# B-R-P/NMSLIB-ZIG

Hardware: AMD Instinct MI355X
Metric: queries/sec @ recall@10, 1M x 128-D L2, batch=1024; HBM GB/s vs peak (higher is better)
Workload: dtype f16+f32

## Files before the change

nmslib_zig_amd/csrc/kernels/bf_kernels.hip:

```cpp
#include <cstdio>
#include <type_traits>
#include <vector>
#include <cstdlib>

#include "common_dev.hpp"
#include "kernels.hpp"

namespace gfxknn {

enum BfMode : int { BF_L2 = 0, BF_DOT = 1, BF_COS = 2, BF_L1 = 3, BF_LINF = 4, BF_COSC = 5, BF_L2D = 6 };

struct BfArgs {
    const float* base;
    const float* aux;
    const float* qaux;
    int aux_stride;
    const float* queries;
    u64* cand;
    int* cand_cnt;
    uint32_t* gthr;
    uint32_t* gq;
    int xj, xm;
    int n, ldb, nqt, nsplit, rows_per_split, kprime, cap;
    int kcs;
// ... 752 lines not shown
            check_block(acc1, 1, t - 1);
        }
        __builtin_amdgcn_sched_barrier(0);
        if (!compute) break;
        const bool more = t + kRing - 1 < nstages;
        if (more && !(a.dbg & 2)) issue_tile(t + kRing - 1);
#pragma unroll
        for (int i = 0; i < 16; ++i) {
            acc0[i] = 0;
            acc1[i] = 0;
        }
#pragma unroll
        for (int ks = 0; ks < 4; ++ks) {
            acc0 = __builtin_amdgcn_mfma_i32_32x32x32_i8(fa[ks], bq[ks], acc0, 0, 0, 0);
            acc1 = __builtin_amdgcn_mfma_i32_32x32x32_i8(fb[ks], bq[ks], acc1, 0, 0, 0);
        }
        if (a.dbg & 1) asm volatile("" ::"v"(acc0[0]), "v"(acc1[0]), "v"(acc0[15]), "v"(acc1[15]));
        if (a.xj > 0 && !(a.dbg & 256) && t > 0 && (((t - 1) & t) == 0 || ((t - 1) & 31) == 31)) exchange_counted();
        if (a.dbg & 8) continue;
        if (more) asm volatile("s_waitcnt vmcnt(12)\n\ts_barrier" ::: "memory");
        else asm volatile("s_waitcnt vmcnt(0)\n\ts_barrier" ::: "memory");
    }
    if (nstages > 0 && !(a.dbg & 1)) {
        if (a.xj > 0 && !(a.dbg & 256)) exchange_counted();
        finish_stage(true);
    }
    if (h == 0) a.cand_cnt[(size_t)qidx * a.nsplit + split] = mycnt;
}

__device__ __forceinline__ uint32_t hit_mask_f32(const f32x16& c, float t) {
    typedef float f32x2 __attribute__((ext_vector_type(2)));
    uint32_t m = 0u;
    const f32x2 tt = {t, t};
#pragma unroll
    for (int i0 = 0; i0 < 16; i0 += 8) {
        f32x2 d[4];
#pragma unroll
        for (int j = 0; j < 4; ++j) d[j] = f32x2{c[i0 + 2 * j], c[i0 + 2 * j + 1]} - tt;
        asm volatile("" : "+v"(d[0]), "+v"(d[1]), "+v"(d[2]), "+v"(d[3]));
#pragma unroll
        for (int j = 0; j < 4; ++j) {
            m = __builtin_amdgcn_alignbit(m, __float_as_uint(d[j][0]), 31);
            m = __builtin_amdgcn_alignbit(m, __float_as_uint(d[j][1]), 31);
        }
    }
    return ~m & 0xffffu;
}
__device__ __forceinline__ uint32_t hit_mask_i32(const i32x16& c, int t) {
    uint32_t m = 0u;
#pragma unroll
    for (int i = 0; i < 16; ++i) m = __builtin_amdgcn_alignbit(m, (uint32_t)(c[i] - t), 31);
    return ~m & 0xffffu;
}
__device__ __forceinline__ void scan_gather_entries(u64* keys, const int* offs, const uint32_t* list, int q, int nl, int caph,
                                                    int tps, int tid, int nthreads) {
    for (int s = tid; s < nl; s += nthreads) {
        const int len = offs[s + 1] - offs[s];
        if (len == 0) continue;
        const uint32_t* e = list + (size_t)q * caph * nl + s;
        const uint32_t row_base = (uint32_t)(s >> 1) * (uint32_t)tps * BF_BN + 4u * (s & 1);
        uint32_t pre[4];
#pragma unroll
        for (int i = 0; i < 4; ++i) pre[i] = (i < len && i < caph) ? e[(size_t)i * nl] : 0u;
        int j = 0;
        auto expand = [&](const uint32_t ent) __attribute__((always_inline)) {
            uint32_t m = ent & 0xffffu;
            const uint32_t r0 = row_base + (ent >> 16) * 32u;
            while (m && j < len) {
                const int bit = 31 - __builtin_clz(m);
                m &= ~(1u << bit);
                const int reg = 15 - bit;
                keys[offs[s] + j++] = (u64)(r0 + (reg & 3) + 8 * (reg >> 2));
            }
        };
#pragma unroll
        for (int i = 0; i < 4; ++i)
            if (i < caph && j < len) expand(pre[i]);
        for (int i = 4; i < caph && j < len; ++i) expand(e[(size_t)i * nl]);
    }
}

struct BfScanArgs {
    const uint8_t* base_i8;
    const int32_t* auxh;
    const uint8_t* queries;
    const int* thr;
    uint32_t* list;
    int* list_cnt;
    int n, nqt, nsplit, tps, caph;
    int tile_stride;
    int* top8;
};

template <int QG, bool SAMPLE>
__global__ __launch_bounds__(256, 2) void bf_scan_u8_kernel(BfScanArgs a) {
    extern __shared__ __attribute__((aligned(16))) char smem[];
    const int tid = threadIdx.x, lane = tid & 63, wave = tid >> 6;
    const int h = lane >> 5, l31 = lane & 31;
    const int b = blockIdx.x;
    const int xcd = b & 7, rest = b >> 3;
    const int qt = rest % a.nqt;
    const int split = (rest / a.nqt) * 8 + xcd;
    if (split >= a.nsplit) return;

    constexpr int kGroup = 4, kRing = 2 * kGroup, kAuxRing = 8, kTileBytes = BF_BN * 128;
    char* ring = smem;
    int* auxr = reinterpret_cast<int*>(ring + kRing * kTileBytes);

    const int tstr = SAMPLE ? a.tile_stride : 1;
    const int tiles_all = (a.n + BF_BN - 1) / BF_BN;
    const int stiles_all = (tiles_all + tstr - 1) / tstr;
    const int nstages = max(0, min(a.tps, stiles_all - split * a.tps));
    const int r_begin = split * a.tps * tstr * BF_BN;
    const int stage_rows = tstr * BF_BN;

    const int dma_row = lane >> 3;
    uint32_t dma_voff[2];
#pragma unroll
    for (int jj = 0; jj < 2; ++jj) {
        const int row = 8 * (2 * wave + jj) + dma_row;
        dma_voff[jj] = (uint32_t)(row * 128 + ((lane & 7) ^ ((row >> 1) & 7)) * 16);
    }
    const uint32_t dma_lds0 = (uint32_t)(uintptr_t)(lptr_t)ring + (uint32_t)(2 * __builtin_amdgcn_readfirstlane(wave) * 1024);
    const uint32_t aux_lds0 = (uint32_t)(uintptr_t)(lptr_t)auxr;
    const uint32_t aux_voff = (uint32_t)lane * 4u;
    auto issue_tile = [&](int stage) __attribute__((always_inline)) {
        const int slot = stage % kRing;
        const int row0 = r_begin + stage * stage_rows;
        const unsigned long long sbase = (unsigned long long)(uintptr_t)a.base_i8 + (unsigned long long)row0 * 128ull;
        const uint32_t m0v = dma_lds0 + (uint32_t)slot * kTileBytes;
#pragma clang diagnostic push
// ... 259 lines not shown
                bsq = __builtin_amdgcn_udot4(bv[u][t], bv[u][t], bsq, false);
                dot = __builtin_amdgcn_udot4(bv[u][t], qv[t], dot, false);
            }
            int d = qsq + bsq - 2 * dot;
            d += __shfl_xor(d, 1, 64);
            d += __shfl_xor(d, 2, 64);
            d += __shfl_xor(d, 4, 64);
            const int j = j0 + 8 * u + g8;
            if (sub == 0 && j < total) keys[j] = ((u64)i32_ord(d) << 32) | pos[u];
        }
    }
    for (int i = total + tid; i < P; i += blockDim.x) keys[i] = ~0ull;
    __syncthreads();
    block_bitonic_u64_asc(keys, P, tid, blockDim.x);
    const int found = total < a.k ? total : a.k;
    for (int i = tid; i < a.k; i += blockDim.x) {
        int32_t id = -1;
        float d = INFINITY;
        if (i < found) {
            const u64 key = keys[i];
            const uint32_t pos = (uint32_t)key;
            id = a.ext_ids ? a.ext_ids[pos] : (int32_t)pos;
            d = (float)ord_i32((uint32_t)(key >> 32));
        }
        a.out_ids[(size_t)q * a.k + i] = id;
        a.out_dists[(size_t)q * a.k + i] = d;
    }
    if (tid == 0 && a.out_cnt) a.out_cnt[q] = found;
}

typedef __bf16 bf16x8 __attribute__((ext_vector_type(8)));
typedef _Float16 f16x8 __attribute__((ext_vector_type(8)));

enum ScanMode : int { SC_L2 = 0, SC_DOT = 1, SC_COS = 2 };

struct BfScanF32Args {
    const __bf16* base_hi;
    const __bf16* base_lo;
    const float* auxp;
    const __bf16* q_hi;
    const __bf16* q_lo;
    const void* base_h16;
    const void* q_h16;
    const float* auxp16;
    int prio_half;
    const float* thr;
    uint32_t* list;
    int* list_cnt;
    int n, nqt, nsplit, tps, caph;
    int tile_stride;
    float* top8;
    const int* group_flag;
    int group_want;
};

#define BF_FRAG_RD(REGS, var, addr) asm volatile("ds_read_b128 %0, %1" : "={" REGS "}"(var) : "v"(addr) : "memory")
#define BF_FRAG_RD_OFF(REGS, var, addr, off) \
    asm volatile("ds_read_b128 %0, %1 offset:%2" : "={" REGS "}"(var) : "v"(addr), "n"(off) : "memory")

template <int MODE, bool SAMPLE, int QG>
__global__ __launch_bounds__(256) void bf_scan_f32_kernel(BfScanF32Args a) {
    constexpr int NW = 4;
    extern __shared__ __attribute__((aligned(16))) char smem[];
    const int tid = threadIdx.x, lane = tid & 63, wave = tid >> 6;
    const int h = lane >> 5, l31 = lane & 31;
    const int b = blockIdx.x;
    const int xcd = b & 7, rest = b >> 3;
    const int qt = rest % a.nqt;
    const int split = (rest / a.nqt) * 8 + xcd;
    if (split >= a.nsplit) return;
    if (a.group_flag && (a.group_flag[qt] != 0) != (a.group_want != 0)) return;

    constexpr int kRing = 4, kAuxRing = 8, kHalfBytes = BF_BN * 256, kStageBytes = 2 * kHalfBytes;
    char* ring = smem;
    float* auxr = reinterpret_cast<float*>(ring + kRing * kStageBytes);

    const int tstr = SAMPLE ? a.tile_stride : 1;
    const int tiles_all = (a.n + BF_BN - 1) / BF_BN;
    const int stiles_all = (tiles_all + tstr - 1) / tstr;
    const int nstages = max(0, min(a.tps, stiles_all - split * a.tps));
    const int r_begin = split * a.tps * tstr * BF_BN;
    const int stage_rows = tstr * BF_BN;

    constexpr int kPieces = 32 / NW;
    static_assert(kPieces == 8, "a wave's pieces lie in one half of the stage");
    const int wave_u = __builtin_amdgcn_readfirstlane(wave);
    uint32_t dma_voff[kPieces];
#pragma unroll
    for (int jj = 0; jj < kPieces; ++jj) {
        const int pj = (kPieces * wave + jj) & 15;
        const int row = 4 * pj + (lane >> 4);
        dma_voff[jj] = (uint32_t)((row * 128 + ((lane & 15) ^ (row & 15)) * 8) * 2);
    }
    const int dma_half = (kPieces * wave_u) >> 4;
    const uint32_t dma_lds0 = (uint32_t)(uintptr_t)(lptr_t)ring + (uint32_t)(dma_half * kHalfBytes + ((kPieces * wave_u) & 15) * 1024);
    const unsigned long long dma_src0 = (unsigned long long)(uintptr_t)(dma_half ? a.base_lo : a.base_hi);
    const uint32_t aux_lds0 = (uint32_t)(uintptr_t)(lptr_t)auxr;
    const uint32_t aux_voff = (uint32_t)lane * 4u;
    auto issue_tile = [&](int stage) __attribute__((always_inline)) {
        const int slot = stage % kRing;
        const int row0 = r_begin + stage * stage_rows;
        const unsigned long long sbase = dma_src0 + (unsigned long long)row0 * 256ull;
        const uint32_t m0v = dma_lds0 + (uint32_t)slot * kStageBytes;
#pragma clang diagnostic push
#pragma clang diagnostic ignored "-Winline-asm"
#pragma unroll
// ... 312 lines not shown
        if constexpr (MODE == SC_COS) return c[i] * ax[(i & 3) + 8 * (i >> 2)];
        else return c[i];
    };
    auto block_max_leaves = [&](const f32x16& c, const float* ax, float (&m)[5]) __attribute__((always_inline)) {
#pragma unroll
        for (int j = 0; j < 5; ++j) {
            if constexpr (MODE == SC_COS)
                m[j] = fmaxf(fmaxf(score_of(c, 3 * j, ax), score_of(c, 3 * j + 1, ax)), score_of(c, 3 * j + 2, ax));
            else
                asm("v_max3_f32 %0, %1, %2, %3" : "=v"(m[j]) : "v"(c[3 * j]), "v"(c[3 * j + 1]), "v"(c[3 * j + 2]));
        }
    };
    auto block_max_root = [&](const f32x16& c, const float* ax, const float (&m)[5]) __attribute__((always_inline)) -> float {
        if constexpr (MODE == SC_COS) {
            return fmaxf(fmaxf(fmaxf(m[0], m[1]), m[2]), fmaxf(fmaxf(m[3], m[4]), score_of(c, 15, ax)));
        } else {
            float r0, r1, r;
            asm("v_max3_f32 %0, %1, %2, %3" : "=v"(r0) : "v"(m[0]), "v"(m[1]), "v"(m[2]));
            asm("v_max3_f32 %0, %1, %2, %3" : "=v"(r1) : "v"(m[3]), "v"(m[4]), "v"(c[15]));
            asm("v_max_f32 %0, %1, %2" : "=v"(r) : "v"(r0), "v"(r1));
            return r;
        }
    };
    auto block_max = [&](const f32x16& c, const float* ax) __attribute__((always_inline)) -> float {
        float m[5];
        block_max_leaves(c, ax, m);
        return block_max_root(c, ax, m);
    };
    auto trigger_of = [&](float m, int g) __attribute__((always_inline)) -> unsigned long long {
        return SAMPLE ? __builtin_amdgcn_ballot_w64(m > thr[g]) : __builtin_amdgcn_ballot_w64(m >= thr[g]);
    };
    auto finish_check = [&](unsigned long long trig, float m, const f32x16& c, int g, const float* ax, int row0) __attribute__((always_inline)) {
        if constexpr (SAMPLE) {
            if (__builtin_expect(trig != 0ull, 0)) {
                float v = (row0 + 32 <= a.n || MODE == SC_L2) ? m : -INFINITY;
#pragma unroll
                for (int j = 0; j < 8; ++j) {
                    const float hi = fmaxf(t8[g][j], v);
                    v = fminf(t8[g][j], v);
                    t8[g][j] = hi;
                }
                thr[g] = t8[g][7];
            }
        } else if (__builtin_expect(trig != 0ull, 0)) {
            uint32_t km;
            if constexpr (MODE == SC_COS) {
                f32x16 sc;
#pragma unroll
                for (int i = 0; i < 16; ++i) sc[i] = score_of(c, i, ax);
                km = hit_mask_f32(sc, thr[g]);
            } else {
                km = hit_mask_f32(c, thr[g]);
            }
            if (row0 + 32 > a.n) {
                int nvalid = a.n - row0;
                asm volatile("" : "+s"(nvalid));
#pragma unroll
                for (int i = 0; i < 16; ++i)
                    if (acc_row(i, h) >= nvalid) km &= ~(0x8000u >> i);
            }
            if (km) {
                if (ecnt[g] < a.caph) lp[g][(size_t)ecnt[g] * (2 * a.nsplit)] = ((uint32_t)(row0 - r_begin) >> 5 << 16) | km;
                ecnt[g]++;
                cnt[g] += __builtin_popcount(km);
            }
        }
    };

    f16x8 fh[4];
    f32x16 iv;
#pragma unroll
    for (int i = 0; i < 16; ++i) iv[i] = 0.f;
    f32x16 acc[2][QG];
#pragma unroll
    for (int g = 0; g < QG; ++g) {
#pragma unroll
        for (int i = 0; i < 16; ++i) {
            acc[0][g][i] = 0.f;
            acc[1][g][i] = -INFINITY;
        }
    }
    const float* pv_ax = auxr;
    int pv_row0 = 0;
    bool have_pv = false;
    float m_pend = 0.f;
    unsigned long long trig_pend = 0ull;
    const uint32_t lds0 = (uint32_t)(uintptr_t)(lptr_t)smem;
    auto load_frag = [&](auto off_tag, int kc) __attribute__((always_inline)) {
        constexpr int OFF = decltype(off_tag)::value;
        const uint32_t ad = vad[kc];
        if constexpr (NW == 4) {
            switch (kc % 4) {
                case 0: BF_FRAG_RD_OFF("v[224:227]", fh[0], ad, OFF); break;
                case 1: BF_FRAG_RD_OFF("v[228:231]", fh[1], ad, OFF); break;
                case 2: BF_FRAG_RD_OFF("v[232:235]", fh[2], ad, OFF); break;
                default: BF_FRAG_RD_OFF("v[236:239]", fh[3], ad, OFF); break;
            }
        } else {
            switch (kc % 4) {
                case 0: BF_FRAG_RD_OFF("v[96:99]", fh[0], ad, OFF); break;
                case 1: BF_FRAG_RD_OFF("v[100:103]", fh[1], ad, OFF); break;
                case 2: BF_FRAG_RD_OFF("v[104:107]", fh[2], ad, OFF); break;
                default: BF_FRAG_RD_OFF("v[108:111]", fh[3], ad, OFF); break;
            }
        }
    };
    using Off0 = std::integral_constant<int, 0>;
    using Off1 = std::integral_constant<int, 32 * 256>;
    auto wait_frag = [&](auto cnt_tag, int kc, bool with_init) __attribute__((always_inline)) {
        constexpr int N = decltype(cnt_tag)::value;
#define BF_W1(STR)                                                                                              \
        if constexpr (NW == 4) {                                                                                \
            switch (kc % 4) {                                                                                   \
                case 0:                                                                                         \
                    if (with_init) asm volatile(STR : "+{v[224:227]}"(fh[0]), "+{v[240:255]}"(iv));             \
// ... 263 lines not shown
#pragma unroll
        for (int i = 0; i < NPER; ++i) {
            const float v = ord_f32(key[i]);
            const bool c = key[i] != 0u && key[i] <= T && v > -INFINITY && t3 - v >= need;
            best = c && key[i] > best ? key[i] : best;
        }
#pragma unroll
        for (int o = 32; o > 0; o >>= 1) {
            const uint32_t other = (uint32_t)__shfl_xor((int)best, o, 64);
            best = other > best ? other : best;
        }
        ok = false;
        if (best != 0u) {
            int above = 0;
#pragma unroll
            for (int i = 0; i < NPER; ++i) above += __popcll(__builtin_amdgcn_ballot_w64(key[i] > best));
            const int jmax = rcap < total ? rcap : total;
            const int j = best == T ? r : above + 1;
            if (j <= jmax) {
                t1 = ord_f32(best);
                ok = true;
            }
        }
    }
    if (lane == 0) {
        thr3[q] = (t3 - 1.02f * e1) / unit;
        thr1[q] = force_precise == 2 ? INFINITY : t1;
        if (!ok) atomicOr(&precise[q / group_q], 1);
    }
}

struct RerankListF32Args {
    const float* base;
    const float* queries;
    const uint32_t* list;
    const int* list_cnt;
    const int32_t* ext_ids;
    int32_t* out_ids;
    float* out_dists;
    int32_t* out_cnt;
    int* tile_fail;
    int n, k, nsplit, caph, p2max, fail_queries, space, dim, ldb;
    int tps;
    const float* queries_sel;
    const float* thr;
    const float* thr1;
    const int* precise;
    int no_split;
    float bmax;
    float bres;
    float scale, scale_q, bres16;
    int sel_dim, sel_ld;
    const float* qaux;
    unsigned long long* prof;
};

__global__ __launch_bounds__(256) void bf_rerank_f32_list_kernel(RerankListF32Args a) {
    const unsigned long long t0 = a.prof ? wall_clock64() : 0;
    auto lap = [&](int i) __attribute__((always_inline)) {
        if (a.prof && threadIdx.x == 0) atomicAdd(&a.prof[i], wall_clock64() - t0);
    };
    extern __shared__ __attribute__((aligned(16))) char smem[];
    u64* keys = reinterpret_cast<u64*>(smem);
    int* offs = reinterpret_cast<int*>(keys + a.p2max);
    __shared__ int s_over, s_split;
    __shared__ float s_qn2, s_e1, s_thr;
    const int q = blockIdx.x, tid = threadIdx.x, lane = tid & 63, wave = tid >> 6;
    const int nl = 2 * a.nsplit;
    if (tid == 0) s_over = 0;
    __syncthreads();
    if (tid < 64) {
        const int per = (nl + 63) / 64;
        int sum = 0, over = 0;
        for (int i = 0; i < per; ++i) {
            const int s = tid * per + i;
            if (s < nl) {
                const int c = a.list_cnt[(size_t)q * nl + s];
                over |= c > a.caph;
                sum += c < a.caph ? c : a.caph;
            }
        }
        int incl = sum;
#pragma unroll
        for (int o = 1; o < 64; o <<= 1) {
            const int v = __shfl_up(incl, o, 64);
            if (tid >= o) incl += v;
        }
        int run = incl - sum;
        for (int i = 0; i < per; ++i) {
            const int s = tid * per + i;
            if (s < nl) {
                offs[s] = run;
                const int c = a.list_cnt[(size_t)q * nl + s];
                run += c < a.caph ? c : a.caph;
            }
        }
        if (tid == 63) offs[nl] = incl;
        if (__any(over != 0) && tid == 0) s_over = 1;
    } else if (wave == 1) {
        const bool split_product = a.precise[q / a.fail_queries] != 0;
        const float* qs = a.queries_sel + (size_t)q * a.sel_ld;
        float ss = 0.f;
        for (int d = lane; d < a.sel_dim; d += 64) ss = fmaf(qs[d], qs[d], ss);
        ss = wave_sum(ss);
        const float e1 = split_product ? 0.f : one_product_error(qs, a.sel_dim, lane, a.scale * (a.space == SP_L2 || a.space == SP_NEGDOT || a.qaux ? a.bmax : 1.0f), a.bres16, a.scale_q);
        if (lane == 0) {
            s_qn2 = ss;
            s_e1 = e1;
            s_split = split_product ? 1 : 0;
            s_thr = split_product ? a.thr[q] : a.thr1[q];
        }
    }
    __syncthreads();
    const int total = offs[nl];
    if ((a.no_split && a.precise[q / a.fail_queries] != 0) ||
        (a.qaux && a.qaux[(size_t)q * 4 + 3] == 0.f)) {
        if (tid == 0) atomicOr(&a.tile_fail[q / a.fail_queries], 1);
        return;
    }
    const int need = a.k < a.n ? a.k : a.n;
    const int want = need + (a.k / 8 > 4 ? a.k / 8 : 4) < a.n ? need + (a.k / 8 > 4 ? a.k / 8 : 4) : a.n;
    if (s_over || total < want || total > a.p2max) {
        if (tid == 0) atomicOr(&a.tile_fail[q / a.fail_queries], 1);
        return;
    }
    lap(0);
    scan_gather_entries(keys, offs, a.list, q, nl, a.caph, a.tps, tid, blockDim.x);
    __syncthreads();
    lap(1);
    const int P = next_pow2(total < 2 ? 2 : total);
    if (a.prof && tid == 0) {
        atomicAdd(&a.prof[8], (unsigned long long)total);
        atomicAdd(&a.prof[9], (unsigned long long)P);
        atomicAdd(&a.prof[10], 1ull);
    }
    const float* qq = a.queries + (size_t)q * a.ldb;
    const int sub = lane & 15, rg = lane >> 4;
    if (a.dim <= 128) {
        float qv[8];
        bool ok[8];
    #pragma unroll
        for (int c = 0; c < 8; ++c) {
            const int d = sub + 16 * c;
            ok[c] = d < a.dim;
            qv[c] = ok[c] ? qq[d] : 0.f;
        }
        constexpr int kU = 4;
        for (int j0 = wave * (4 * kU); j0 < total; j0 += 16 * kU) {
            uint32_t pos[kU];
            float xv[kU][8];
    #pragma unroll
            for (int u = 0; u < kU; ++u) {
                const int j = j0 + 4 * u + rg;
                pos[u] = (uint32_t)keys[j < total ? j : total - 1];
                const float* row = a.base + (size_t)pos[u] * a.ldb + sub;
    #pragma unroll
                for (int c = 0; c < 8; ++c) xv[u][c] = ok[c] ? row[16 * c] : 0.f;
            }
            __builtin_amdgcn_wave_barrier();
    #pragma unroll
            for (int u = 0; u < kU; ++u) {
                float p0[4], p1[4], p2[4];
    #pragma unroll
                for (int v = 0; v < 4; ++v) {
                    p0[v] = p1[v] = p2[v] = 0.f;
    #pragma unroll
                    for (int c = 0; c < 2; ++c) {
                        if (64 * c >= a.dim) continue;
                        const float x = xv[u][v + 4 * c], y = qv[v + 4 * c];
                        if (a.space == SP_L2) {
                            const float t = x - y;
                            p0[v] = fmaf(t, t, p0[v]);
                        } else {
                            p0[v] = fmaf(x, y, p0[v]);
                            if (a.space != SP_NEGDOT) {
                                p1[v] = fmaf(x, x, p1[v]);
                                p2[v] = fmaf(y, y, p2[v]);
                            }
                        }
                    }
                }
                auto tree = [&](const float* p) __attribute__((always_inline)) -> float {
                    float s = (p[0] + p[2]) + (p[1] + p[3]);
    #pragma unroll
                    for (int o = 8; o > 0; o >>= 1) s += __shfl_xor(s, o, 64);
                    return s;
                };
// ... 82 lines not shown
    }
    __syncthreads();
    lap(2);
    if (total <= 512 && a.k <= 32) {
        __shared__ u64 s_head[128];
        const int e0 = wave * 128 + 2 * lane;
        u64 k0 = e0 < total ? keys[e0] : ~0ull, k1 = e0 + 1 < total ? keys[e0 + 1] : ~0ull;
        wave_sort128_u64(k0, k1, lane);
        if (lane < 16) {
            s_head[wave * 32 + 2 * lane] = k0;
            s_head[wave * 32 + 2 * lane + 1] = k1;
        }
        __syncthreads();
        if (wave == 0) {
            k0 = s_head[2 * lane];
            k1 = s_head[2 * lane + 1];
            wave_sort128_u64(k0, k1, lane);
            if (lane < 16) {
                keys[2 * lane] = k0;
                keys[2 * lane + 1] = k1;
            }
        }
        __syncthreads();
    } else {
        for (int i = total + tid; i < P; i += blockDim.x) keys[i] = ~0ull;
        __syncthreads();
        block_bitonic_u64_asc(keys, P, tid, blockDim.x);
    }
    lap(3);
    const int found = total < a.k ? total : a.k;
    if (total < a.n) {
        const bool split_product = s_split != 0;
        if (tid == 0) {
            const float qn2 = s_qn2, qn = sqrtf(qn2);
            const float dk = ord_f32((uint32_t)(keys[found - 1] >> 32));
            float sk, e, extra = 0.f;
            if (a.qaux) {
                const float sh = sinf(0.5f * dk);
                const float omc = a.space == SP_ANGULAR ? 2.0f * sh * sh : dk;
                const float qnorm = a.qaux[(size_t)q * 4 + 2];
                sk = -omc * qnorm;
                e = 6.1036e-5f * qn * a.bmax;
                extra = 1e-6f * qn * a.bmax + 2e-6f * qnorm;
            } else if (a.space == SP_L2) {
                sk = 0.5f * (qn2 - dk * dk);
                e = 6.1036e-5f * qn * a.bmax;
            } else if (a.space == SP_NEGDOT) {
                sk = -dk;
                e = 6.1036e-5f * qn * a.bmax;
            } else {
                sk = (a.space == SP_ANGULAR ? cosf(dk) : 1.0f - dk) * qn;
                e = 6.1036e-5f * qn;
            }
            const float t = s_thr;
            if (!split_product) {
                const float unit = a.scale * a.scale_q;
                sk *= unit;
                extra *= unit;
                e = s_e1;
            }
            e += extra + 1e-6f * (fabsf(sk) + fabsf(t));
            if (!(sk - t >= e)) atomicOr(&a.tile_fail[q / a.fail_queries], 1);
        }
    }
    lap(4);
    for (int i = tid; i < a.k; i += blockDim.x) {
        int32_t id = -1;
        float d = INFINITY;
        if (i < found) {
            const u64 key = keys[i];
            const uint32_t pos = (uint32_t)key;
            id = a.ext_ids ? a.ext_ids[pos] : (int32_t)pos;
            d = ord_f32((uint32_t)(key >> 32));
        }
        a.out_ids[(size_t)q * a.k + i] = id;
        a.out_dists[(size_t)q * a.k + i] = d;
    }
    if (tid == 0 && a.out_cnt) a.out_cnt[q] = found;
    lap(5);
}

__global__ void row_maxnorm_kernel(const float* rows, int n, int ld, int dim, int relative, unsigned* out_bits, float scale16) {
    const int lane = threadIdx.x & 63;
    const int wpb = blockDim.x >> 6;
    float mb = 0.f, mr = 0.f, ma = 0.f, mh = 0.f;
    for (int row = blockIdx.x * wpb + (threadIdx.x >> 6); row < n; row += gridDim.x * wpb) {
        const float* p = rows + (size_t)row * ld;
        float s = 0.f, r = 0.f, rh = 0.f;
        for (int d = lane; d < dim; d += 64) {
            const float v = p[d], w = v - (float)(__bf16)v;
            const float vs = scale16 * v, wh = vs - (float)(_Float16)vs;
            s = fmaf(v, v, s);
            r = fmaf(w, w, r);
            rh = fmaf(wh, wh, rh);
            ma = fmaxf(ma, fabsf(v));
        }
        s = wave_sum(s);
        r = wave_sum(r);
        rh = wave_sum(rh);
        const float nb = sqrtf(s), nr = sqrtf(r), nh = sqrtf(rh);
        mb = fmaxf(mb, nb);
        mr = fmaxf(mr, relative ? (nb > 0.f ? nr / nb : 0.f) : nr);
        mh = fmaxf(mh, relative ? (nb > 0.f ? nh / nb : 0.f) : nh);
    }
    ma = wave_max(ma);
    if (lane == 0) {
        atomicMax(out_bits, __float_as_uint(mb));
// ... 929 lines not shown
}

template <int MODE, bool SAMPLE, int QG>
static hipError_t launch_scan_f32_one(const BfScanF32Args& a, int grid, size_t lds, hipStream_t s) {
    hipError_t e = hipFuncSetAttribute(reinterpret_cast<const void*>(bf_scan_f32_kernel<MODE, SAMPLE, QG>),
                                       hipFuncAttributeMaxDynamicSharedMemorySize, (int)lds);
    if (e != hipSuccess) return e;
    hipLaunchKernelGGL((bf_scan_f32_kernel<MODE, SAMPLE, QG>), dim3(grid), dim3(256), lds, s, a);
    return hipGetLastError();
}
template <int MODE, bool SAMPLE, int QG, int NW>
static hipError_t launch_scan_bf16_one(const BfScanF32Args& a, int grid, size_t lds, hipStream_t s) {
    hipError_t e = hipFuncSetAttribute(reinterpret_cast<const void*>(bf_scan_bf16_kernel<MODE, SAMPLE, QG, NW>),
                                       hipFuncAttributeMaxDynamicSharedMemorySize, (int)lds);
    if (e != hipSuccess) return e;
    hipLaunchKernelGGL((bf_scan_bf16_kernel<MODE, SAMPLE, QG, NW>), dim3(grid), dim3(NW * 64), lds, s, a);
    return hipGetLastError();
}
template <int MODE>
static hipError_t launch_scan_f32_mode(const BfScanF32Args& a, bool sample, int terms, int qg, int grid, size_t lds, hipStream_t s, int kch = 1) {
    if (kch > 1) {
        if (terms != 1) return hipSuccess;
        auto go = [&](auto kern) -> hipError_t {
            hipError_t e = hipFuncSetAttribute(reinterpret_cast<const void*>(kern), hipFuncAttributeMaxDynamicSharedMemorySize, (int)lds);
            if (e != hipSuccess) return e;
            hipLaunchKernelGGL(kern, dim3(grid), dim3(256), lds, s, a);
            return hipGetLastError();
        };
        switch (kch) {
            case 2: return sample ? go(bf_scan_bf16_kernel<MODE, true, 1, 4, 2>) : go(bf_scan_bf16_kernel<MODE, false, 1, 4, 2>);
            case 3: return sample ? go(bf_scan_bf16_kernel<MODE, true, 1, 4, 3>) : go(bf_scan_bf16_kernel<MODE, false, 1, 4, 3>);
            case 4: return sample ? go(bf_scan_bf16_kernel<MODE, true, 1, 4, 4>) : go(bf_scan_bf16_kernel<MODE, false, 1, 4, 4>);
            case 6: return sample ? go(bf_scan_bf16_kernel<MODE, true, 1, 4, 6>) : go(bf_scan_bf16_kernel<MODE, false, 1, 4, 6>);
            case 8: return sample ? go(bf_scan_bf16_kernel<MODE, true, 1, 4, 8>) : go(bf_scan_bf16_kernel<MODE, false, 1, 4, 8>);
            default: return hipErrorInvalidValue;
        }
    }
    const char* w8e = getenv("NMSLIB_GPU_BF16_W8");
    const int w8 = w8e ? atoi(w8e) : 7;
    if (sample) return (w8 & 4) ? launch_scan_bf16_one<MODE, true, 1, 8>(a, grid, lds, s) : launch_scan_bf16_one<MODE, true, 2, 4>(a, grid, lds, s);
    if (terms == 1) {
        if (qg == 2) return (w8 & 1) ? launch_scan_bf16_one<MODE, false, 2, 8>(a, grid, lds, s) : launch_scan_bf16_one<MODE, false, 4, 4>(a, grid, lds, s);
        return (w8 & 2) ? launch_scan_bf16_one<MODE, false, 1, 8>(a, grid, lds, s) : launch_scan_bf16_one<MODE, false, 2, 4>(a, grid, lds, s);
    }
    if (qg == 2) return launch_scan_f32_one<MODE, false, 4>(a, grid, lds, s);
    return launch_scan_f32_one<MODE, false, 2>(a, grid, lds, s);
}

static void dump_rerank_list_clocks(const unsigned long long* d_prof, hipStream_t s) {
    unsigned long long h[16];
    (void)hipStreamSynchronize(s);
    (void)hipMemcpy(h, d_prof, sizeof(h), hipMemcpyDeviceToHost);
    const double wg = h[10] ? (double)h[10] : 1.0;
    fprintf(stderr, "[rerank f32 list] workgroups %llu rows/query %.1f P %.1f | us since start: prefix %.2f gather %.2f distances %.2f "
            "sort %.2f proof %.2f out %.2f\n", h[10], h[8] / wg, h[9] / wg, h[0] / wg / 100, h[1] / wg / 100, h[2] / wg / 100,
            h[3] / wg / 100, h[4] / wg / 100, h[5] / wg / 100);
}

static void dump_f32_fast_checksums(const BfF32Fast& f, const BfFastWs& ws, hipStream_t s) {
    (void)hipStreamSynchronize(s);
    auto sum = [&](const void* d, size_t bytes) -> unsigned long long {
        std::vector<uint32_t> h(bytes / 4);
        (void)hipMemcpy(h.data(), d, bytes, hipMemcpyDeviceToHost);
        unsigned long long x = 1469598103934665603ull;
        for (uint32_t v : h) x = (x ^ v) * 1099511628211ull;
        return x;
    };
    std::vector<int> cnt((size_t)f.qpad * f.nsplit * 2);
    (void)hipMemcpy(cnt.data(), ws.list_cnt, cnt.size() * 4, hipMemcpyDeviceToHost);
    std::vector<uint32_t> lst((size_t)f.qpad * f.nsplit * 2 * f.caph);
    (void)hipMemcpy(lst.data(), ws.list, lst.size() * 4, hipMemcpyDeviceToHost);
    unsigned long long lx = 1469598103934665603ull;
    long long rows = 0;
    const size_t nl = (size_t)f.nsplit * 2;
    for (size_t i = 0; i < cnt.size(); ++i) {
        rows += cnt[i];
        int have = 0;
        for (int j = 0; j < f.caph && have < cnt[i]; ++j) {
            const uint32_t e = lst[((i / nl) * f.caph + j) * nl + i % nl];
            lx = (lx ^ e) * 1099511628211ull;
            have += __builtin_popcount(e & 0xffffu);
        }
    }
    fprintf(stderr, "[f32fast] top8 %016llx thr %016llx thr1 %016llx flags %016llx cnt %016llx list %016llx rows %lld\n",
            sum(ws.top8, bf_fast_ws_bytes(f).top8), sum(ws.thr, (size_t)f.qpad * 4), sum(ws.thr1(f), (size_t)f.qpad * 4),
            sum(ws.tile_fail(f), (size_t)f.nqt * 8), sum(ws.list_cnt, cnt.size() * 4), lx, rows);
}

hipError_t launch_bf_f32_fast(const BfF32Fast& f, int space, int nq, int k, const BfF32Rows& rows, const BfF32Tiles& tiles,
                              const BfF32Queries& q, const BfFastWs& ws, const BfOut& out, const BfScanEvents& ev,
                              hipStream_t s) {
    const int sdim = f.cosc ? f.sel_dim : rows.dim, sld = f.cosc ? q.sel_ld : rows.ldb;
    float* top8 = static_cast<float*>(ws.top8);
    float* thr = static_cast<float*>(ws.thr);
    float* thr1 = ws.thr1(f);
    int* tile_fail = ws.tile_fail(f);
    int* precise = ws.precise(f);
    void* q_hi = ws.q_tile(f, BfFastWs::Q_HI);
    void* q_lo = ws.q_tile(f, BfFastWs::Q_LO);
    void* q_h16 = ws.q_tile(f, BfFastWs::Q_H16);
    hipError_t e;
    {
        const BfPlan& fb = f.fallback;
        uint32_t* gthr = reinterpret_cast<uint32_t*>(ws.fb.cnt + (size_t)fb.qpad * fb.nsplit);
        const size_t gwords = 2 * ((size_t)fb.qpad + (size_t)fb.qpad * fb.nsplit);
        size_t work = (size_t)f.qpad * f.dp > gwords ? (size_t)f.qpad * f.dp : gwords;
        size_t grid = (work + 255) / 256;
        if (grid > 2048) grid = 2048;
        hipLaunchKernelGGL(bf_f32_prep_kernel, dim3((unsigned)grid), dim3(256), 0, s, q.raw, nq, sdim, q.sel, f.qpad,
// ... 2 lines not shown
                           tile_fail, 2 * f.nqt, ws.flags_fb, fb.nqt, gthr, gwords, f.dp, static_cast<_Float16*>(q_h16), q.scale_q);
        e = hipGetLastError();
        if (e != hipSuccess) return e;
    }
    auto scan = [&](const BfScanF32Args& sa, bool sample, int terms, int grid) -> hipError_t {
        const size_t lds = terms == 1 ? f.lds_scan1 : f.lds_scan;
        if (f.mode == 0) return launch_scan_f32_mode<SC_L2>(sa, sample, terms, f.qg, grid, lds, s, f.kch);
        if (f.mode == 1) return launch_scan_f32_mode<SC_DOT>(sa, sample, terms, f.qg, grid, lds, s, f.kch);
        return launch_scan_f32_mode<SC_COS>(sa, sample, terms, f.qg, grid, lds, s, f.kch);
    };
    BfScanF32Args a{};
    a.base_hi = static_cast<const __bf16*>(tiles.hi);
    a.base_lo = static_cast<const __bf16*>(tiles.lo);
    a.auxp = tiles.auxp;
    a.q_hi = static_cast<const __bf16*>(q_hi);
    a.q_lo = static_cast<const __bf16*>(q_lo);
    a.base_h16 = tiles.h16;
    {
        static const int prio = getenv("NMSLIB_GPU_BF16_PRIO") ? atoi(getenv("NMSLIB_GPU_BF16_PRIO")) : 0;
        a.prio_half = prio;
    }
    a.q_h16 = q_h16;
    a.auxp16 = tiles.auxp16;
    a.n = rows.n;
    a.nqt = f.nqt;
    BfScanF32Args sa = a;
    sa.nqt = f.qpad / (f.kch > 1 ? 128 : 256);
    sa.nsplit = f.s_nsplit;
    sa.tps = f.s_tps;
    sa.tile_stride = f.stride;
    sa.top8 = top8;
    e = scan(sa, true, 1, 8 * sa.nqt * (f.s_nsplit / 8));
    if (e != hipSuccess) return e;
    {
        static const bool dbg_nohit = getenv("NMSLIB_GPU_DEBUG") && (atoi(getenv("NMSLIB_GPU_DEBUG")) & 8192);
        const int depth = f.rcap <= 64 && f.s_nsplit >= 32 ? 4 : 8;
        const dim3 tgrid((f.qpad + 3) / 4);
#define BF_THR_ARGS                                                                                                               \
    top8, 2 * f.s_nsplit, depth, f.r, f.rcap, nq, f.qpad, q.sel, sld, sdim, tiles.scale * (f.mode == 2 ? 1.0f : tiles.bmax), tiles.bres16, f.tq, \
        f.force_precise ? 1 : (dbg_nohit ? 2 : 0), thr, thr1, precise, q.scale_q, tiles.scale * q.scale_q
        if (2 * f.s_nsplit * depth <= 512) hipLaunchKernelGGL(bf_f32_threshold_kernel<8>, tgrid, dim3(256), 0, s, BF_THR_ARGS);
        else hipLaunchKernelGGL(bf_f32_threshold_kernel<16>, tgrid, dim3(256), 0, s, BF_THR_ARGS);
#undef BF_THR_ARGS
    }
    e = hipGetLastError();
    if (e != hipSuccess) return e;
    a.list = ws.list;
    a.list_cnt = ws.list_cnt;
    a.nsplit = f.nsplit;
    a.tps = f.tps;
    a.caph = f.caph;
    a.tile_stride = 1;
    a.group_flag = precise;
    const int grid = 8 * f.nqt * (f.nsplit / 8);
    if (ev.first) (void)hipEventRecord(ev.first, s);
    if (!f.force_precise) {
        a.thr = thr1;
        a.group_want = 0;
        e = scan(a, false, 1, grid);
        if (e != hipSuccess) return e;
    }
    a.thr = thr;
    a.group_want = 1;
    e = scan(a, false, 3, grid);
    if (ev.second) (void)hipEventRecord(ev.second, s);
    if (e != hipSuccess) return e;
    RerankListF32Args r{};
    r.base = rows.orig;
    r.queries = q.padded;
    r.list = ws.list;
    r.list_cnt = ws.list_cnt;
    r.ext_ids = out.ext_ids;
    r.out_ids = out.ids;
    r.out_dists = out.dists;
    r.out_cnt = out.cnt;
    r.tile_fail = tile_fail;
    r.n = rows.n;
    r.k = k;
    r.nsplit = f.nsplit;
    r.caph = f.caph;
    r.tps = f.tps;
    r.p2max = f.p2max;
    r.fail_queries = f.tq;
    r.no_split = f.kch > 1 ? 1 : 0;
    r.space = space;
    r.dim = rows.dim;
    r.ldb = rows.ldb;
    r.queries_sel = q.sel;
    r.sel_dim = sdim;
    r.sel_ld = sld;
    r.scale = tiles.scale;
    r.scale_q = q.scale_q;
    r.bres16 = tiles.bres16;
    r.qaux = f.cosc ? q.qaux_cosc : nullptr;
    r.thr = thr;
    r.thr1 = thr1;
    r.precise = precise;
    r.bmax = tiles.bmax;
    r.bres = tiles.bres;
    static const int dbg = getenv("NMSLIB_GPU_DEBUG") ? atoi(getenv("NMSLIB_GPU_DEBUG")) : 0;
    static unsigned long long* d_prof = nullptr;
    if (dbg & 4096) {
        if (!d_prof) (void)hipMalloc(&d_prof, 16 * 8);
        (void)hipMemsetAsync(d_prof, 0, 16 * 8, s);
        r.prof = d_prof;
    }
    e = hipFuncSetAttribute(reinterpret_cast<const void*>(bf_rerank_f32_list_kernel),
                            hipFuncAttributeMaxDynamicSharedMemorySize, (int)f.lds_rerank);
    if (e != hipSuccess) return e;
    hipLaunchKernelGGL(bf_rerank_f32_list_kernel, dim3(nq), dim3(256), f.lds_rerank, s, r);
    e = hipGetLastError();
    if (e != hipSuccess) return e;
    if (dbg & 4096) dump_rerank_list_clocks(d_prof, s);
    if (dbg & 2048) dump_f32_fast_checksums(f, ws, s);
    BfF32Queries fq = q;
    fq.sel = f.cosc ? q.centred : q.sel;
    fq.qaux_cosc = f.cosc ? q.qaux_cosc : nullptr;
    return launch_bf_adaptive_f32(f.fallback, space, k, rows, fq, ws.fb, ws.flags_fb, BfGate{tile_fail, f.tq / 128}, out, s,
                                  true);
}

hipError_t launch_row_aux_f32(const float* base, int n, int ldb, int dim, int space, float* aux,
                              hipStream_t s) {
    if (n == 0) return hipSuccess;
    hipLaunchKernelGGL(row_aux_f32_kernel, dim3((n + 3) / 4), dim3(256), 0, s, base, n, ldb, dim, space, aux);
    return hipGetLastError();
}
hipError_t launch_prepare_u8(const uint8_t* base, int n, uint8_t* rows_i8, int32_t* aux, int32_t* auxh, hipStream_t s) {
    const int n_pad = bf_u8_rows_padded(n);
    hipLaunchKernelGGL(prepare_u8_kernel, dim3((n_pad + 3) / 4), dim3(256), 0, s, base, n, n_pad, rows_i8, aux, auxh);
    return hipGetLastError();
}
hipError_t launch_pad_rows(const void* src, int rows, int dim, void* dst, int rows_pad, int ld,
                           int elem_bytes, hipStream_t s) {
    const size_t total = (size_t)rows_pad * ld * elem_bytes;
    if (total == 0) return hipSuccess;
    int grid = (int)((total + 255) / 256);
    if (grid > 4096) grid = 4096;
    hipLaunchKernelGGL(pad_rows_kernel, dim3(grid), dim3(256), 0, s, (const uint8_t*)src, rows,
                       dim * elem_bytes, (uint8_t*)dst, rows_pad, ld * elem_bytes);
    return hipGetLastError();
}
hipError_t launch_normalize_rows(float* rows, int n, int ld, int dim, hipStream_t s) {
    if (n == 0) return hipSuccess;
    hipLaunchKernelGGL(normalize_rows_kernel, dim3((n + 3) / 4), dim3(256), 0, s, rows, n, ld, dim);
    return hipGetLastError();
}
hipError_t launch_row_aux_cosc(const float* orig, const float* centred, int n, int ldb, int dim, double mu_norm, float* aux,
                               hipStream_t s) {
    if (n == 0) return hipSuccess;
// ... 71 lines not shown
```

nmslib_zig_amd/csrc/kernels/kernels.hpp:

```cpp
#pragma once
#include <hip/hip_runtime_api.h>
#include <stddef.h>
#include <stdint.h>

#include <utility>

namespace gfxknn {

enum SpaceCode : int {
    SP_L2 = 0,
    SP_L1 = 1,
    SP_LINF = 2,
    SP_COSINE = 3,
    SP_ANGULAR = 4,
    SP_NEGDOT = 5,
    SP_L2SQR_SIFT = 6,
    SP_L2SQR = 7,
    SP_NORMCOS = 8,
    SP_QNORM_NEGDOT = 9,
    SP_LEVEN = 10,
    SP_BIT_HAMMING = 11,
    SP_KLDIV = 12,
    SP_KLDIV_RQ = 13,
    SP_KLDIVGEN = 14,
// ... 88 lines not shown
                               const BfCand& c, const BfGate& gate, hipStream_t s, bool cleared = false);
hipError_t launch_bf_select_direct_f32(const BfPlan& p, int space, const float* base, const float* queries_padded,
                                       const BfCand& c, const BfGate& gate, hipStream_t s,
                                       bool cleared_second_region = false);
hipError_t launch_bf_rerank(const BfPlan& p, int space, int dim, int k, const void* base, const void* queries_padded,
                            const BfCand& c, const BfGate& gate, const BfVerify& verify, const BfOut& out, hipStream_t s);
hipError_t launch_bf_adaptive_f32(const BfPlan& p, int space, int k, const BfF32Rows& rows, const BfF32Queries& q,
                                  const BfCand& c, int* flags, const BfGate& gate, const BfOut& out, hipStream_t s,
                                  bool cleared = false);

struct BfU8Fast {
    bool use;
    int qg;
    int qpad, nqt;
    int stride, r;
    int nsplit, tps, caph;
    int p2max;
    size_t lds_scan, lds_thr, lds_rerank;
    int s_nsplit, s_tps;
    BfPlan fallback;
};
BfU8Fast bf_u8_fast_plan(int n, int nq, int k);

struct BfF32Fast {
    bool use;
    int mode;
    int qg;
    bool cosc;
    int sel_dim;
    int kch;
    int dp;
    int tq;
    int qpad, nqt;
    int stride, r;
    int rcap;
    bool force_precise;
    int nsplit, tps, caph, p2max;
    int s_nsplit, s_tps;
    size_t lds_scan, lds_scan1, lds_thr, lds_rerank;
    BfPlan fallback;
};
BfF32Fast bf_f32_fast_plan(int n, int dim, int nq, int k, int space, bool cosine_centred);

struct BfFastWsBytes {
    size_t top8, thr, list, list_cnt, cand, cnt, flags_fb, queries;
};
inline BfFastWsBytes bf_fast_ws_bytes(const BfU8Fast& f) {
    const size_t lists = (size_t)f.qpad * f.nsplit * 2;
    return {(size_t)f.qpad * f.s_nsplit * 2 * 8 * 4, (size_t)f.qpad * 4 + (size_t)f.nqt * 4 + 64, lists * f.caph * 4, lists * 4,
            bf_cand_elems(f.fallback) * 8, bf_cnt_elems(f.fallback) * 4, 0, 0};
}
inline BfFastWsBytes bf_fast_ws_bytes(const BfF32Fast& f) {
    const size_t lists = (size_t)f.qpad * f.nsplit * 2;
    return {(size_t)f.qpad * f.s_nsplit * 2 * 8 * 4, (size_t)f.qpad * 8 + (size_t)f.nqt * 8 + 64, lists * f.caph * 4, lists * 4,
            bf_cand_elems(f.fallback) * 8, bf_cnt_elems(f.fallback) * 4, (size_t)f.fallback.nqt * 4 + 64,
            (size_t)f.qpad * f.dp * 2 * 3};
}
struct BfFastWs {
    void* top8;
    void* thr;
    uint32_t* list;
    int* list_cnt;
    BfCand fb;
    int* flags_fb;
    void* queries;

    int* tile_fail(const BfU8Fast& f) const { return static_cast<int*>(thr) + f.qpad; }
    float* thr1(const BfF32Fast& f) const { return static_cast<float*>(thr) + f.qpad; }
    int* tile_fail(const BfF32Fast& f) const { return reinterpret_cast<int*>(thr1(f) + f.qpad); }
    int* precise(const BfF32Fast& f) const { return tile_fail(f) + f.nqt; }
    enum QueryTile { Q_HI = 0, Q_LO = 1, Q_H16 = 2 };
    void* q_tile(const BfF32Fast& f, QueryTile t) const { return static_cast<char*>(queries) + (size_t)t * f.qpad * f.dp * 2; }
};

hipError_t launch_bf_u8_fast(const BfU8Fast& f, int nq, int k, const BfU8Rows& rows, const uint8_t* queries_raw,
                             uint8_t* queries_padded, const BfFastWs& ws, const BfOut& out, const BfScanEvents& ev,
                             hipStream_t s);

inline int bf_f32_rows_padded(int n) { return (n + BF_BN - 1) / BF_BN * BF_BN + BF_BN; }
hipError_t launch_row_maxnorm(const float* rows, int n, int ld, int dim, bool relative_residual, float* out, hipStream_t s,
                              float scale16 = 0.f);
struct BfF32Tiles {
    void *hi, *lo;
    float* auxp;
    void* h16;
    float* auxp16;
    float scale, bres16;
    int dp;
    float bmax, bres;
};
struct BfSplitSrc {
    const float* rows;
    int n, n_pad, ld, cols;
};
hipError_t launch_split_bf16(const BfSplitSrc& src, const float* aux, float aux_pad, float aux16_mul, const BfF32Tiles& dst,
                             hipStream_t s);
hipError_t launch_bf_f32_fast(const BfF32Fast& f, int space, int nq, int k, const BfF32Rows& rows, const BfF32Tiles& tiles,
                              const BfF32Queries& q, const BfFastWs& ws, const BfOut& out, const BfScanEvents& ev,
                              hipStream_t s);
hipError_t launch_row_aug_cosc(const float* orig, const float* centred, int n, int ldb, int dim, double mu_norm, float lambda,
                               float* out, int ldo, int* zero_rows, hipStream_t s);
hipError_t launch_query_aug_cosc(const float* centred, const float* qaux, int nq, int qpad, int ldb, int dim, float lambda,
                                 float* out, int ldo, hipStream_t s);

hipError_t launch_pair_distance(int space, const void* a, const void* b, int dim, float* out,
                                hipStream_t s);

struct HnswDeviceGraph {
    const void* rows;
    const int32_t* row_norm;
    const int32_t* links0;
    const int64_t* up_off;
    const int32_t* up_links;
    const int32_t* ext_ids;
    int n, dim, ldv;
    int maxM, maxM0, maxlevel, enterpoint;
    int space;
    int normalize_query;
};
// ... 220 lines not shown
```

Measured before the change: 2.851 million.

## Store per-entry max score in scan lists and prune rerank rows below bound

The f32 scan kernel now writes, next to each hit-mask entry, the best approximate score of that 32-row block into a second list plane, which doubles the list workspace. In the non-split rerank path the gather tags each entry's first key with that max. A wave then finds the r-th largest entry max, derives a cutoff with an error margin, and compacts away rows whose block max falls below it before exact distances are computed. This aims to cut the rows fetched and reranked per query, at the cost of extra list writes in the scan, a selection pass, and a tighter threshold that could affect recall if the margin is wrong.

```diff
diff --git a/nmslib_zig_amd/csrc/kernels/bf_kernels.hip b/nmslib_zig_amd/csrc/kernels/bf_kernels.hip
--- a/nmslib_zig_amd/csrc/kernels/bf_kernels.hip
+++ b/nmslib_zig_amd/csrc/kernels/bf_kernels.hip
@@ -828,31 +828,38 @@
     for (int i = 0; i < 16; ++i) m = __builtin_amdgcn_alignbit(m, (uint32_t)(c[i] - t), 31);
     return ~m & 0xffffu;
 }
+constexpr uint32_t kEntryHead = 0x80000000u;
+template <bool TWO_WORDS = false>
 __device__ __forceinline__ void scan_gather_entries(u64* keys, const int* offs, const uint32_t* list, int q, int nl, int caph,
-                                                    int tps, int tid, int nthreads) {
+                                                    int tps, int tid, int nthreads, size_t m_off = 0) {
     for (int s = tid; s < nl; s += nthreads) {
         const int len = offs[s + 1] - offs[s];
         if (len == 0) continue;
         const uint32_t* e = list + (size_t)q * caph * nl + s;
         const uint32_t row_base = (uint32_t)(s >> 1) * (uint32_t)tps * BF_BN + 4u * (s & 1);
-        uint32_t pre[4];
-#pragma unroll
-        for (int i = 0; i < 4; ++i) pre[i] = (i < len && i < caph) ? e[(size_t)i * nl] : 0u;
+        uint32_t pre[4], prem[TWO_WORDS ? 4 : 1];
+#pragma unroll
+        for (int i = 0; i < 4; ++i) {
+            pre[i] = (i < len && i < caph) ? e[(size_t)i * nl] : 0u;
+            if constexpr (TWO_WORDS) prem[i] = (i < len && i < caph) ? e[(size_t)i * nl + m_off] : 0u;
+        }
         int j = 0;
-        auto expand = [&](const uint32_t ent) __attribute__((always_inline)) {
+        auto expand = [&](const uint32_t ent, const uint32_t emax) __attribute__((always_inline)) {
             uint32_t m = ent & 0xffffu;
             const uint32_t r0 = row_base + (ent >> 16) * 32u;
+            u64 hi = TWO_WORDS ? ((u64)f32_ord(__uint_as_float(emax)) << 32) | kEntryHead : 0ull;
             while (m && j < len) {
                 const int bit = 31 - __builtin_clz(m);
                 m &= ~(1u << bit);
                 const int reg = 15 - bit;
-                keys[offs[s] + j++] = (u64)(r0 + (reg & 3) + 8 * (reg >> 2));
+                keys[offs[s] + j++] = hi | (u64)(r0 + (reg & 3) + 8 * (reg >> 2));
+                hi &= ~(u64)kEntryHead;
             }
         };
 #pragma unroll
         for (int i = 0; i < 4; ++i)
-            if (i < caph && j < len) expand(pre[i]);
-        for (int i = 4; i < caph && j < len; ++i) expand(e[(size_t)i * nl]);
+            if (i < caph && j < len) expand(pre[i], TWO_WORDS ? prem[i] : 0u);
+        for (int i = 4; i < caph && j < len; ++i) expand(e[(size_t)i * nl], TWO_WORDS ? e[(size_t)i * nl + m_off] : 0u);
     }
 }
 
@@ -1218,6 +1225,7 @@
     float* top8;
     const int* group_flag;
     int group_want;
+    size_t list_m_off;
 };
 
 #define BF_FRAG_RD(REGS, var, addr) asm volatile("ds_read_b128 %0, %1" : "={" REGS "}"(var) : "v"(addr) : "memory")
@@ -1636,15 +1644,24 @@
             } else {
                 km = hit_mask_f32(c, thr[g]);
             }
+            float em = block_max(c, ax);
             if (row0 + 32 > a.n) {
                 int nvalid = a.n - row0;
                 asm volatile("" : "+s"(nvalid));
 #pragma unroll
                 for (int i = 0; i < 16; ++i)
                     if (acc_row(i, h) >= nvalid) km &= ~(0x8000u >> i);
+                em = -INFINITY;
+#pragma unroll
+                for (int i = 0; i < 16; ++i)
+                    if (km & (0x8000u >> i)) em = fmaxf(em, score_of(c, i, ax));
             }
             if (km) {
-                if (ecnt[g] < a.caph) lp[g][(size_t)ecnt[g] * (2 * a.nsplit)] = ((uint32_t)(row0 - r_begin) >> 5 << 16) | km;
+                if (ecnt[g] < a.caph) {
+                    uint32_t* ep = lp[g] + (size_t)ecnt[g] * (2 * a.nsplit);
+                    ep[0] = ((uint32_t)(row0 - r_begin) >> 5 << 16) | km;
+                    ep[a.list_m_off] = __float_as_uint(em);
+                }
                 ecnt[g]++;
                 cnt[g] += __builtin_popcount(km);
             }
@@ -2014,8 +2031,22 @@
     float scale, scale_q, bres16;
     int sel_dim, sel_ld;
     const float* qaux;
+    size_t list_m_off;
     unsigned long long* prof;
 };
+
+template <int NPER>
+__device__ __forceinline__ uint32_t entry_rth_largest(const u64* keys, int total, int r, int lane, uint32_t t_ord) {
+    uint32_t key[NPER];
+#pragma unroll
+    for (int i = 0; i < NPER; ++i) {
+        const int j = i * 64 + lane;
+        const u64 kv = j < total ? keys[j] : 0ull;
+        const uint32_t hi = (uint32_t)(kv >> 32);
+        key[i] = ((uint32_t)kv & kEntryHead) ? (hi == 0xFF800000u ? t_ord : hi) : 0u;
+    }
+    return wave_rth_largest_u32<NPER>(key, r);
+}
 
 __global__ __launch_bounds__(256) void bf_rerank_f32_list_kernel(RerankListF32Args a) {
     const unsigned long long t0 = a.prof ? wall_clock64() : 0;
@@ -2025,8 +2056,8 @@
     extern __shared__ __attribute__((aligned(16))) char smem[];
     u64* keys = reinterpret_cast<u64*>(smem);
     int* offs = reinterpret_cast<int*>(keys + a.p2max);
-    __shared__ int s_over, s_split;
-    __shared__ float s_qn2, s_e1, s_thr;
+    __shared__ int s_over, s_split, s_rows;
+    __shared__ float s_qn2, s_e1, s_thr, s_cut;
     const int q = blockIdx.x, tid = threadIdx.x, lane = tid & 63, wave = tid >> 6;
     const int nl = 2 * a.nsplit;
     if (tid == 0) s_over = 0;
@@ -2074,7 +2105,8 @@
         }
     }
     __syncthreads();
-    const int total = offs[nl];
+    const int listed = offs[nl];
+    int total = listed;
     if ((a.no_split && a.precise[q / a.fail_queries] != 0) ||
         (a.qaux && a.qaux[(size_t)q * 4 + 3] == 0.f)) {
         if (tid == 0) atomicOr(&a.tile_fail[q / a.fail_queries], 1);
@@ -2087,14 +2119,45 @@
         return;
     }
     lap(0);
-    scan_gather_entries(keys, offs, a.list, q, nl, a.caph, a.tps, tid, blockDim.x);
-    __syncthreads();
+    if (s_split) {
+        scan_gather_entries(keys, offs, a.list, q, nl, a.caph, a.tps, tid, blockDim.x);
+        __syncthreads();
+        if (tid == 0) s_cut = -INFINITY;
+    } else {
+        scan_gather_entries<true>(keys, offs, a.list, q, nl, a.caph, a.tps, tid, blockDim.x, a.list_m_off);
+        __syncthreads();
+        uint32_t kap = 0u;
+        const uint32_t t_ord = f32_ord(s_thr);
+        if (total <= 256) kap = entry_rth_largest<4>(keys, total, want, lane, t_ord);
+        else if (total <= 1024) kap = entry_rth_largest<16>(keys, total, want, lane, t_ord);
+        const float kappa = ord_f32(kap);
+        const float cut = (kap != 0u && fabsf(kappa) < INFINITY) ? kappa - 2.1f * s_e1 : -INFINITY;
+        __syncthreads();
+        if (wave == 0) {
+            int w = 0;
+            for (int j0 = 0; j0 < total; j0 += 64) {
+                const int j = j0 + lane;
+                const u64 kv = j < total ? keys[j] : 0ull;
+                const bool keep = j < total && !(ord_f32((uint32_t)(kv >> 32)) < cut);
+                const unsigned long long bal = __builtin_amdgcn_ballot_w64(keep);
+                if (keep) keys[w + __popcll(bal & ((1ull << lane) - 1ull))] = (u64)((uint32_t)kv & ~kEntryHead);
+                w += __popcll(bal);
+            }
+            if (lane == 0) {
+                s_rows = w;
+                s_cut = w < total ? cut : -INFINITY;
+            }
+        }
+        __syncthreads();
+        total = s_rows;
+    }
     lap(1);
     const int P = next_pow2(total < 2 ? 2 : total);
     if (a.prof && tid == 0) {
-        atomicAdd(&a.prof[8], (unsigned long long)total);
+        atomicAdd(&a.prof[8], (unsigned long long)listed);
         atomicAdd(&a.prof[9], (unsigned long long)P);
         atomicAdd(&a.prof[10], 1ull);
+        atomicAdd(&a.prof[11], (unsigned long long)total);
     }
     const float* qq = a.queries + (size_t)q * a.ldb;
     const int sub = lane & 15, rg = lane >> 4;
@@ -2283,7 +2346,7 @@
                 sk = (a.space == SP_ANGULAR ? cosf(dk) : 1.0f - dk) * qn;
                 e = 6.1036e-5f * qn;
             }
-            const float t = s_thr;
+            const float t = fmaxf(s_thr, s_cut);
             if (!split_product) {
                 const float unit = a.scale * a.scale_q;
                 sk *= unit;
@@ -3319,9 +3382,9 @@
     (void)hipStreamSynchronize(s);
     (void)hipMemcpy(h, d_prof, sizeof(h), hipMemcpyDeviceToHost);
     const double wg = h[10] ? (double)h[10] : 1.0;
-    fprintf(stderr, "[rerank f32 list] workgroups %llu rows/query %.1f P %.1f | us since start: prefix %.2f gather %.2f distances %.2f "
-            "sort %.2f proof %.2f out %.2f\n", h[10], h[8] / wg, h[9] / wg, h[0] / wg / 100, h[1] / wg / 100, h[2] / wg / 100,
-            h[3] / wg / 100, h[4] / wg / 100, h[5] / wg / 100);
+    fprintf(stderr, "[rerank f32 list] workgroups %llu rows/query %.1f fetched/query %.1f P %.1f | us since start: prefix %.2f "
+            "gather %.2f distances %.2f sort %.2f proof %.2f out %.2f\n", h[10], h[8] / wg, h[11] / wg, h[9] / wg, h[0] / wg / 100,
+            h[1] / wg / 100, h[2] / wg / 100, h[3] / wg / 100, h[4] / wg / 100, h[5] / wg / 100);
 }
 
 static void dump_f32_fast_checksums(const BfF32Fast& f, const BfFastWs& ws, hipStream_t s) {
@@ -3430,6 +3493,7 @@
     a.caph = f.caph;
     a.tile_stride = 1;
     a.group_flag = precise;
+    a.list_m_off = ws.list_m_off(f);
     const int grid = 8 * f.nqt * (f.nsplit / 8);
     if (ev.first) (void)hipEventRecord(ev.first, s);
     if (!f.force_precise) {
@@ -3474,6 +3538,7 @@
     r.thr = thr;
     r.thr1 = thr1;
     r.precise = precise;
+    r.list_m_off = ws.list_m_off(f);
     r.bmax = tiles.bmax;
     r.bres = tiles.bres;
     static const int dbg = getenv("NMSLIB_GPU_DEBUG") ? atoi(getenv("NMSLIB_GPU_DEBUG")) : 0;
diff --git a/nmslib_zig_amd/csrc/kernels/kernels.hpp b/nmslib_zig_amd/csrc/kernels/kernels.hpp
--- a/nmslib_zig_amd/csrc/kernels/kernels.hpp
+++ b/nmslib_zig_amd/csrc/kernels/kernels.hpp
@@ -164,7 +164,7 @@
 }
 inline BfFastWsBytes bf_fast_ws_bytes(const BfF32Fast& f) {
     const size_t lists = (size_t)f.qpad * f.nsplit * 2;
-    return {(size_t)f.qpad * f.s_nsplit * 2 * 8 * 4, (size_t)f.qpad * 8 + (size_t)f.nqt * 8 + 64, lists * f.caph * 4, lists * 4,
+    return {(size_t)f.qpad * f.s_nsplit * 2 * 8 * 4, (size_t)f.qpad * 8 + (size_t)f.nqt * 8 + 64, 2 * lists * f.caph * 4, lists * 4,
             bf_cand_elems(f.fallback) * 8, bf_cnt_elems(f.fallback) * 4, (size_t)f.fallback.nqt * 4 + 64,
             (size_t)f.qpad * f.dp * 2 * 3};
 }
@@ -177,6 +177,7 @@
     int* flags_fb;
     void* queries;
 
+    size_t list_m_off(const BfF32Fast& f) const { return (size_t)f.qpad * f.caph * f.nsplit * 2; }
     int* tile_fail(const BfU8Fast& f) const { return static_cast<int*>(thr) + f.qpad; }
     float* thr1(const BfF32Fast& f) const { return static_cast<float*>(thr) + f.qpad; }
     int* tile_fail(const BfF32Fast& f) const { return reinterpret_cast<int*>(thr1(f) + f.qpad); }
```

Result: faster. 2.988 million (median of 6 runs) (+4.8%).
